# vseib/point-cloud-donkey

Hardware: AMD Instinct MI355X
Metric: objects/sec classified (ModelNet10-like, SHOT-352) (higher is better)
Workload: dtype f32; 1 GPU; configs[1]: ModelNet10-like test split, 16384 pts, 1024 uniform keypoints/object, SHOT-352 (Radius 0.4, LRF 0.3), exact kNN K=1 squared-L2, mean-shift bandwidth 0.6; points_per_object=16384, keypoints_per_object=1024, classes=10, codebook_words=102400, descriptor_dim=352, collective_world_size=1

## Files before the change

### point-cloud-donkey_amd/csrc/codebook.hip

```cpp
#include "common.h"
#include <cstring>
#include <cmath>
#include <limits>

int ism_codebook_split_bf16(ismhip_ctx* ctx, ismhip_codebook* cb, uint32_t absmax_bits);
int ism_codebook_build_pca(ismhip_ctx* ctx, ismhip_codebook* cb);
void ism_codebook_free_pca(ismhip_codebook* cb);

namespace {

__global__ void k_word_norms(const float* __restrict__ words, int n_words, int n_words_pad, int dim_pad, float* __restrict__ norm) {
    const int row = blockIdx.x * 4 + (threadIdx.x >> 6);
    if (row >= n_words_pad) return;
    const int lane = lane_id();
    float s = 0.f;
    for (int c = lane; c < dim_pad; c += 64) { const float v = words[(size_t)row * dim_pad + c]; s += v * v; }
    s = wave_sum_f(s);
    if (lane == 0) norm[row] = row < n_words ? s : __builtin_inff();
}

__global__ void k_sqrt_permuted(const float* __restrict__ src, const uint32_t* __restrict__ perm, int n_words, int dim_pad, float* __restrict__ dst, size_t n) {
    const size_t i = (size_t)blockIdx.x * blockDim.x + threadIdx.x;
    if (i >= n) return;
    const size_t row = i / dim_pad; const int col = (int)(i % dim_pad);
// ... 140 lines not shown
            uint32_t b; memcpy(&b, &words_h[i], 4);
            if (!(words_h[i] >= 0.f)) nonneg = false;
            b &= 0x7fffffffu; amax = b > amax ? b : amax;
        }
        cb->words_nonneg = nonneg;
        int rc = ism_codebook_split_bf16(ctx, cb, amax);
        if (rc != ISMHIP_OK || hipStreamSynchronize(ctx->stream) != hipSuccess) return fail(rc != ISMHIP_OK ? rc : ISMHIP_ERR_HIP, "codebook_create: bf16 split");
        if (!ctx->codebook_light) rc = ism_codebook_build_pca(ctx, cb);
        if (rc != ISMHIP_OK || hipStreamSynchronize(ctx->stream) != hipSuccess) return fail(rc != ISMHIP_OK ? rc : ISMHIP_ERR_HIP, "codebook_create: rotated image");
        if (nonneg && dim > 64 && ctx->knn_hellinger && n_words >= 1024 && !ctx->codebook_light) {
            ismhip_codebook* sh = new ismhip_codebook();
            cb->chi_shadow = sh;
            sh->n_words = n_words; sh->dim = dim; sh->dim_pad = cb->dim_pad; sh->n_words_pad = cb->n_words_pad; sh->n_classes = n_classes;
            if (hipMalloc((void**)&sh->words, wbytes) != hipSuccess || hipMalloc((void**)&sh->word_norm, (size_t)cb->n_words_pad * 4) != hipSuccess)
                return fail(ISMHIP_ERR_NOMEM, "codebook_create: sqrt image");
            std::vector<uint32_t> perm(n_words);
            for (int i = 0; i < n_words; ++i) perm[i] = (uint32_t)i;
            uint64_t st = 0x9E3779B97F4A7C15ull ^ (uint64_t)n_words;
            for (int i = n_words - 1; i > 0; --i) {
                st += 0x9E3779B97F4A7C15ull; uint64_t z = st; z = (z ^ (z >> 30)) * 0xBF58476D1CE4E5B9ull; z = (z ^ (z >> 27)) * 0x94D049BB133111EBull; z ^= z >> 31;
                std::swap(perm[i], perm[(size_t)(z % (uint64_t)(i + 1))]);
            }
            if (!upload(&sh->shadow_perm, perm.data(), (size_t)n_words)) return fail(ISMHIP_ERR_NOMEM, "codebook_create: sqrt image permutation");
            const size_t tot = (size_t)cb->n_words_pad * cb->dim_pad;
            hipLaunchKernelGGL(k_sqrt_permuted, dim3((unsigned)((tot + 255) / 256)), dim3(256), 0, ctx->stream, cb->words, sh->shadow_perm, n_words, cb->dim_pad, sh->words, tot);
            hipLaunchKernelGGL(k_word_norms, dim3((cb->n_words_pad + 3) / 4), dim3(256), 0, ctx->stream, sh->words, n_words, cb->n_words_pad, cb->dim_pad, sh->word_norm);
            if (hipGetLastError() != hipSuccess || hipStreamSynchronize(ctx->stream) != hipSuccess) return fail(ISMHIP_ERR_HIP, "codebook_create: sqrt image kernels");
            std::vector<float> nh(n_words);
            if (hipMemcpy(nh.data(), sh->word_norm, (size_t)n_words * 4, hipMemcpyDeviceToHost) != hipSuccess) return fail(ISMHIP_ERR_HIP, "codebook_create: sqrt norms copy");
            float mx = 0.f;
            for (float v : nh) if (v > mx || v != v) mx = v;
            sh->max_norm2 = mx;
            float amaxf; memcpy(&amaxf, &amax, 4);
            const float samax = sqrtf(amaxf);
            uint32_t samax_bits; memcpy(&samax_bits, &samax, 4);
            rc = ism_codebook_split_bf16(ctx, sh, samax_bits);
            if (rc != ISMHIP_OK || hipStreamSynchronize(ctx->stream) != hipSuccess) return fail(rc != ISMHIP_OK ? rc : ISMHIP_ERR_HIP, "codebook_create: sqrt 16-bit images");
// ... 95 lines not shown
```

### point-cloud-donkey_amd/csrc/common.h

```cpp
#pragma once
#include <hip/hip_runtime.h>
#include <stdint.h>
#include <map>
#include <set>
#include <string>
#include <vector>
#include "../../include/ismhip.h"

#define ISM_WAVE 64

#define ISM_GRID_MAXDIM 32
#define ISM_GRID_MAXCELLS (ISM_GRID_MAXDIM * ISM_GRID_MAXDIM * ISM_GRID_MAXDIM)
#define ISM_GRID_STRIDE (ISM_GRID_MAXCELLS + 1)

#define ISM_GRID_XFRAC 3
struct GridMeta {
    float minv[3];
    float cell[3];
    float inv_cell[3];
    int   dim[3];
    float centroid[3];
    uint32_t n_finite;
};

// ... 47 lines not shown
    float max_norm2 = 0.f;
    float* word_weight = nullptr;
    uint32_t* vote_off = nullptr;
    float* vote_xyz = nullptr;
    float* vote_weight = nullptr;
    float* vote_class_weight = nullptr;
    uint32_t* vote_class = nullptr;
    uint32_t* vote_instance = nullptr;
    float* vote_bbox_quat = nullptr;
    float* vote_bbox_size = nullptr;
    float* class_sigma = nullptr;
    uint32_t* word_class = nullptr;
    ismhip_codebook* chi_shadow = nullptr;
    uint32_t* shadow_perm = nullptr;
    PcaImage pca, pca2;
};

struct TimerAcc {
    std::vector<std::pair<hipEvent_t, hipEvent_t>> pending;
    double ms = 0.0;
    int64_t launches = 0;
};

struct ismhip_ctx {
    int device = 0;
    hipStream_t stream = nullptr;
    bool own_stream = false;
    std::string err;
    bool timers_on = false;
    std::map<std::string, TimerAcc> timers;
    std::vector<hipEvent_t> event_pool;
    struct Slot { void* p = nullptr; size_t bytes = 0; };
    std::map<int, Slot> scratch;
    float* lut_srgb = nullptr;
    float* lut_sxyz = nullptr;
    std::vector<ismhip_cloud*> cloud_pool;
    uint32_t* truncated_d = nullptr;
    uint32_t knn_stats[2] = {0, 0};
    std::set<const void*> attr_done;
    uint32_t knn_stage2_queries = 0;
    bool knn_two_stage = true;
    bool knn_small_tile = false;
    bool knn_join = true;
    bool knn_qpanel2 = true;
    bool knn_qpanel = false;
    bool knn_half = false;
    bool knn_ring32 = false;
    int knn_splits = 0;
    int knn_t = 0;
    int knn_dbg = 0;
    bool knn_no_ring = false;
    bool knn_kb32 = false;
    bool xcd_map = true;
    float grid_xfrac = 0.f;
    int shot_var = 0;
    bool knn_hell_emit = true;
    bool knn_hellinger = true;
    int knn_t1 = 2;
    int knn_pre_step = 32;
    float knn_pre_gamma = 1.0f;
    bool knn_prepass = true;
    int knn_pca_m = -1;
    bool knn_stage2_t4 = false;
    bool codebook_light = false;
    int knn_pca_m2 = -1;
    uint32_t knn_pca_launches = 0;
    uint32_t knn_thr_overflow = 0;
    uint32_t knn_thr_mfma_launches = 0;
    int knn_mode = 0;
};

enum ScratchSlot {
    SCR_KP_OFF = 1, SCR_TIE_LIST, SCR_TIE_REC, SCR_TIE_KEYS, SCR_COUNTERS, SCR_KNN_CAND_IDX, SCR_KNN_CAND_VAL,
    SCR_QNORM, SCR_FPFH_FLAG, SCR_FPFH_LIST, SCR_FPFH_SPFH, SCR_FPFH_LOOKUP, SCR_SLOT_OFF, SCR_CLASS_BW,
    SCR_COMPACT_KEEP, SCR_COMPACT_POS, SCR_OBJ_COUNT, SCR_QPAD, SCR_LRF_COV, SCR_KNN_FLAGS, SCR_KNN_QSPLIT, SCR_MAX_REC, SCR_QNORM2, SCR_KNN_Q2, SCR_KNN_LIST2, SCR_TRAIN, SCR_TRAIN2, SCR_MAX_WORK, SCR_KMEANS, SCR_KNN_CLOCK, SCR_PCA, SCR_KNN_THR0, SCR_KNN_QSQRT, SCR_KNN_HELL_EMIT, SCR_KNN_THR, SCR_KNN_THR2, SCR_TRAIN_ACT
};
// ... 245 lines not shown
```

### point-cloud-donkey_amd/csrc/ctx.hip

```cpp
#include "common.h"
#include <cmath>
#include <cstring>
#include <cstdlib>

extern "C" void ism_cloud_pool_release(ismhip_ctx* ctx);

int ism_set_err(ismhip_ctx* ctx, int code, const std::string& msg) {
    if (ctx) ctx->err = msg;
    return code;
}

void* ism_scratch(ismhip_ctx* ctx, int slot, size_t bytes) {
    if (bytes == 0) bytes = 16;
    auto& s = ctx->scratch[slot];
    if (s.bytes >= bytes) return s.p;
    if (s.p) { (void)hipStreamSynchronize(ctx->stream); (void)hipFree(s.p); s.p = nullptr; s.bytes = 0; }
    size_t want = bytes + bytes / 4;
    void* p = nullptr;
    if (hipMalloc(&p, want) != hipSuccess) { ism_set_err(ctx, ISMHIP_ERR_NOMEM, "scratch hipMalloc failed"); return nullptr; }
    s.p = p; s.bytes = want;
    return p;
}

TimerScope::TimerScope(ismhip_ctx* c, const char* n) : ctx(c), name(n) {
// ... 45 lines not shown
    { const char* e = getenv("ISMHIP_KNN_HALF"); ctx->knn_half = e && e[0] == '1'; }
    { const char* e = getenv("ISMHIP_KNN_RING32"); ctx->knn_ring32 = e && e[0] == '1'; }
    { const char* e = getenv("ISMHIP_KNN_SPLITS"); ctx->knn_splits = e ? atoi(e) : 0; }
    { const char* e = getenv("ISMHIP_KNN_T"); ctx->knn_t = e ? atoi(e) : 0; }
    { const char* e = getenv("ISMHIP_KNN_DBG"); ctx->knn_dbg = e ? atoi(e) : 0; }
    { const char* e = getenv("ISMHIP_KNN_NORING"); ctx->knn_no_ring = e && e[0] == '1'; }
    { const char* e = getenv("ISMHIP_KNN_KB32"); ctx->knn_kb32 = e && e[0] == '1'; }
    { const char* e = getenv("ISMHIP_KNN_HELL_EMIT"); ctx->knn_hell_emit = !(e && e[0] == '0'); }
    { const char* e = getenv("ISMHIP_KNN_HELLINGER"); ctx->knn_hellinger = !(e && e[0] == '0'); }
    { const char* e = getenv("ISMHIP_KNN_T1"); if (e) ctx->knn_t1 = atoi(e); }
    { const char* e = getenv("ISMHIP_KNN_STAGE2_T4"); if (e) ctx->knn_stage2_t4 = atoi(e) != 0; }
    { const char* e = getenv("ISMHIP_KNN_PRE_STEP"); if (e && atoi(e) > 0) ctx->knn_pre_step = atoi(e); }
    { const char* e = getenv("ISMHIP_KNN_PRE_GAMMA"); if (e) ctx->knn_pre_gamma = (float)atof(e); }
    { const char* e = getenv("ISMHIP_KNN_PREPASS"); ctx->knn_prepass = !(e && e[0] == '0'); }
    { const char* e = getenv("ISMHIP_KNN_PCA_M"); ctx->knn_pca_m = e ? atoi(e) : -1; }
    { const char* e = getenv("ISMHIP_KNN_PCA_M2"); ctx->knn_pca_m2 = e ? atoi(e) : -1; }
    { const char* e = getenv("ISMHIP_KNN_TILE128"); ctx->knn_small_tile = e && e[0] == '1'; }
    if (!own) { ctx->stream = (hipStream_t)stream; ctx->own_stream = false; }
    else {
        if (hipStreamCreateWithFlags(&ctx->stream, hipStreamNonBlocking) != hipSuccess) { delete ctx; return ISMHIP_ERR_HIP; }
        ctx->own_stream = true;
    }
    std::vector<float> srgb(256), sxyz(4000);
    for (int i = 0; i < 256; i++) {
        float f = static_cast<float>(i) / 255.0f;
        srgb[i] = (f > 0.04045) ? powf((f + 0.055f) / 1.055f, 2.4f) : f / 12.92f;
    }
    for (int i = 0; i < 4000; i++) {
        float f = static_cast<float>(i) / 4000.0f;
        sxyz[i] = (f > 0.008856) ? static_cast<float>(powf(f, 0.3333f)) : static_cast<float>((7.787 * f) + (16.0 / 116.0));
// ... 94 lines not shown
```

### point-cloud-donkey_amd/csrc/knn.hip

```cpp
#include "common.h"

int ism_pca_rotate_queries(ismhip_ctx* ctx, const ismhip_codebook* cb, const PcaImage* P, const float* q, int nq, int ldq, unsigned short* dst);

namespace {

typedef float f32x16 __attribute__((ext_vector_type(16)));
typedef float f32x4 __attribute__((ext_vector_type(4)));

#define KNN_BM 128
#define KNN_BN 128
#define KNN_BK 32
#define KNN_LDK 36

template <int T>
struct TopT {
    float v[T]; int i[T];
    __device__ __forceinline__ void init() {
#pragma unroll
        for (int t = 0; t < T; ++t) { v[t] = __builtin_inff(); i[t] = -1; }
    }
    __device__ __forceinline__ void push_flat(float x, int idx) {
        bool c[T];
#pragma unroll
        for (int t = 0; t < T; ++t) c[t] = x < v[t];
// ... 1202 lines not shown
        uint32_t ibase = 0;
        if (lane == 0) {
            const uint32_t qs = atomicAdd(&flag_count[0], 1u);
            ibase = atomicAdd(&flag_count[1], (uint32_t)nv);
            qrec[3 * (size_t)qs] = (uint32_t)qi; qrec[3 * (size_t)qs + 1] = ibase; qrec[3 * (size_t)qs + 2] = (uint32_t)nv;
        }
        ibase = __shfl(ibase, 0, 64);
        if (viol) {
            const uint32_t it = ibase + __popcll(vmask & ((1ull << lane) - 1ull));
            items[2 * (size_t)it] = (uint32_t)qi; items[2 * (size_t)it + 1] = (uint32_t)lane;
        }
    }
}
__global__ __launch_bounds__(256) void k_knn_rerank_pca(const float* __restrict__ words, int dim, int dim_pad, int n_words,
                                                        const float* __restrict__ q, int nq, int ldq,
                                                        const int* __restrict__ cand_idx, const float* __restrict__ cand_val, int cand_stride, int n_cand,
                                                        const float* __restrict__ cand_bound, int n_bound, PcaVerify pv,
                                                        int k, int32_t* __restrict__ idx_out, float* __restrict__ dist_out,
                                                        uint32_t* __restrict__ flag_count, uint32_t* __restrict__ qrec, uint32_t* __restrict__ items) {
    const int qi = blockIdx.x * 4 + (threadIdx.x >> 6);
    if (qi >= nq) return;
    const int lane = lane_id();
    const float* qp = q + (size_t)qi * ldq;
    float qn2 = 0.f;
    for (int i = lane; i < dim; i += 64) { const float v = qp[i]; qn2 += v * v; }
    qn2 = wave_sum_f(qn2);
    float qn2h = 0.f;
    {
        const size_t tile = (size_t)(qi >> 8); const int r = qi & 255;
        for (int i = lane; i < pv.nk * 32; i += 64) {
// ... 3 lines not shown
        qn2h = wave_sum_f(qn2h) * pv.inv_sq2;
    }
    const float dlt = pv.d_rel * (sqrtf(qn2) * 1.00001f) + pv.dq_abs + pv.dc;
    const float eps_s = (pv.eps_c2 + pv.dot2 * sqrtf(qn2h * pv.cmax2)) * 1.00001f;
    auto lb_of = [&](float s) -> float {
        float L = qn2h * (1.f - 16.f * KNN_U) + s - eps_s;
        L -= 4.f * KNN_U * (qn2h + fabsf(s));
        if (!(L > 0.f)) return 0.f;
        const float t = sqrtf(L) * (1.f - 4.f * KNN_U) - dlt;
        if (!(t > 0.f)) return 0.f;
        return t * t * pv.inv_sig2 * (1.f - 8.f * KNN_U);
    };
    int id = -1; float av = __builtin_inff();
    if (lane < n_cand) { id = cand_idx[(size_t)qi * cand_stride + lane]; av = cand_val[(size_t)qi * cand_stride + lane]; }
    if (!(id >= 0 && id < n_words)) { id = -1; av = __builtin_inff(); }
    const float lb = id >= 0 ? lb_of(av) : __builtin_inff();
    bool done = id < 0;
    unsigned long long key = ~0ull;
    {
        __shared__ __attribute__((aligned(16))) float s_terms[4][1344];
        float* sT = s_terms[threadIdx.x >> 6];
        float kth = __builtin_inff(); int n_eval = 0;
        for (;;) {
            const float cur = done ? __builtin_inff() : lb;
            const float mn = wave_min_f(cur);
            if (!(mn < __builtin_inff())) break;
            if (n_eval >= k && mn * (1.f - pv.ku) > kth) break;
            const unsigned long long eq = __ballot(!done && cur == mn);
            const int src = __ffsll((long long)eq) - 1;
            const int cid = __shfl(id, src, 64);
// ... 164 lines not shown

#define KNN_FB_UNITS 8192u
__host__ __device__ inline uint32_t knn_fb_parts(uint32_t n_items) {
    if (n_items == 0 || n_items > KNN_FB_UNITS / 2) return 1u;
    const uint32_t p = KNN_FB_UNITS / n_items;
    return p > 256u ? 256u : p;
}
#define KNN_MAX_K 16
#define KNN_FB_MAXJ 84
template <int KM>
__global__ __launch_bounds__(256) void k_knn_fallback(const float* __restrict__ words, int dim, int dim_pad, int n_words,
                                                      const float* __restrict__ q, int ldq, int metric, int k, int tiles_per_split, int n_tiles,
                                                      int tile_rows, int wr_rows ,
                                                      const uint32_t* __restrict__ flag_count, const uint32_t* __restrict__ items,
                                                      const int32_t* __restrict__ idx_in, const float* __restrict__ dist_in,
                                                      unsigned long long* __restrict__ item_out, size_t part_base) {
    __shared__ __attribute__((aligned(16))) float s_terms[4][1344];
    const int lane = threadIdx.x & 63;
    const int g = lane >> 4, l16 = lane & 15;
    const uint32_t n_items = flag_count[1];
    const bool l2 = metric != ISMHIP_METRIC_CHI2;
    const bool lay_all = l2 && wr_rows == -2;
    const bool lay16 = l2 && wr_rows == -1;
    const bool lay16h = l2 && wr_rows == -3;
    const int rows_per_tile = lay_all ? tile_rows : ((lay16 || lay16h) ? 32 : (l2 ? wr_rows / 2 : tile_rows));
    const int nj = dim_pad / 16;
    const uint32_t gw = blockIdx.x * 4 + (threadIdx.x >> 6), nw = gridDim.x * 4;
    const uint32_t P = knn_fb_parts(n_items);
    unsigned long long* outp = P > 1 ? item_out + KM * part_base : item_out;
    for (uint32_t u = gw; u < n_items * P; u += nw) {
        const uint32_t it = u / P, part_i = u % P;
// ... 8 lines not shown
        for (int j = 0; j < KM; ++j) best[j] = ~0ull;
        float thr = __builtin_inff();
        {
            const int id = idx_in[(size_t)qi * k + (k - 1)];
            if (id >= 0) thr = dist_in[(size_t)qi * k + (k - 1)];
        }
        const int steps = (total + 3) / 4;
        const int e_beg = 4 * (int)((long long)steps * part_i / P), e_end = min(total, 4 * (int)((long long)steps * (part_i + 1) / P));
        for (int e0 = e_beg; e0 < e_end; e0 += 4) {
            const int e = e0 + g;
            int r = n_words;
            if (e < e_end) {
                const int tile = mt0 + e / rows_per_tile, y = e % rows_per_tile;
                const int x = lay_all ? y : ((lay16 || lay16h) ? (wr * 128 + ((y >> 2) << 4) + (fq << 2) + (y & 3)) : (l2 ? (wr * wr_rows + (((y >> 2) << 3) | (h << 2) | (y & 3))) : y));
                r = tile * tile_rows + x;
            }
            float part = 0.f;
            if (r < n_words) {
                const float* wp = words + (size_t)r * dim_pad;
                if (!l2) { for (int j = 0; j < nj; ++j) { const int i = l16 + 16 * j; const float a = i < dim ? qp[i] : 0.f, c = wp[i], sm = a + c, df = a - c; part += sm > 0.f ? df * df / sm : 0.f; } }
                else { for (int j = 0; j < nj; ++j) { const int i = l16 + 16 * j; const float df = (i < dim ? qp[i] : 0.f) - wp[i]; part += df * df; } }
            }
#pragma unroll
            for (int o = 8; o > 0; o >>= 1) part += __shfl_xor(part, o, 64);
            const bool hit = r < n_words && !(part > thr * 1.0001f + 1e-30f);
            unsigned long long hm = __ballot(hit && l16 == 0);
            while (hm) {
                const int src = __ffsll((long long)hm) - 1; hm &= hm - 1;
                const int rr = __shfl(r, src, 64);
                const float d = wave_functor(metric, qp, words + (size_t)rr * dim_pad, dim, lane, s_terms[threadIdx.x >> 6]);
// ... 79 lines not shown
    const float a = d3[i * 3], b = d3[i * 3 + 1], c = d3[i * 3 + 2];
    int id = -1; float dd = __builtin_nanf("");
    if (i2 < 0) {
        if (i0 >= 0) { id = i0; dd = a; }
    } else {
        const uint32_t c0 = word_class[i0], c1 = word_class[i1], c2 = word_class[i2];
        if (c0 == c1 && c0 == c2) { id = i0; dd = a; }
        else if (c0 == c1 && c0 != c2) { if (a / c < thr) { id = i0; dd = a; } }
        else if (c0 != c1 && c1 == c2) { if (a / b >= thr) { id = i1; dd = b; } }
        else if (c0 != c1 && c1 != c2) { if (a / b < thr) { id = i0; dd = a; } }
    }
    idx_out[i] = id; dist_out[i] = dd;
}

struct KnnStage1 { uint32_t* flag_count; uint32_t* qrec; };
template <int T>
int run_knn(ismhip_ctx* ctx, const ismhip_codebook* cb, int metric, int nq, const float* q, int k,
            int32_t* idx_out, float* dist_out, KnnStage1* stage1 = nullptr, const char* tname = nullptr, bool many_splits = false, int use_pca = 0 , const float* hell_q = nullptr) {
    const bool hell = hell_q != nullptr && metric == ISMHIP_METRIC_CHI2 && cb->chi_shadow;
    const ismhip_codebook* xb = hell ? cb->chi_shadow : cb;
    const int cmetric = hell ? ISMHIP_METRIC_L2SQ : metric;
    if (cb->dim_pad / 16 > KNN_FB_MAXJ) return ism_set_err(ctx, ISMHIP_ERR_UNSUPPORTED, "knn: descriptor longer than 1344 not built");
    const float* qq = q; int ldq = cb->dim;
    if (cb->dim_pad != cb->dim) {
        float* qpad = (float*)ism_scratch(ctx, SCR_QPAD, (size_t)nq * cb->dim_pad * sizeof(float));
        if (!qpad) return ISMHIP_ERR_NOMEM;
        const size_t tot = (size_t)nq * cb->dim_pad;
        hipLaunchKernelGGL(k_pad_rows, dim3((unsigned)((tot + 255) / 256)), dim3(256), 0, ctx->stream, q, nq, cb->dim, qpad, cb->dim_pad);
        ISM_CHECK_LAUNCH(ctx, "k_pad_rows");
        qq = qpad; ldq = cb->dim_pad;
// ... 109 lines not shown
                    default: break;
                } else
                switch (ctx->knn_dbg) {
                    case 1: rk = (const void*)k_knn_l2_ring<T, 1>; break;  case 3: rk = (const void*)k_knn_l2_ring<T, 3>; break;
                    case 5: rk = (const void*)k_knn_l2_ring<T, 5>; break;  case 7: rk = (const void*)k_knn_l2_ring<T, 7>; break;
                    case 9: rk = (const void*)k_knn_l2_ring<T, 9>; break;  case 13: rk = (const void*)k_knn_l2_ring<T, 13>; break;
                    case 15: rk = (const void*)k_knn_l2_ring<T, 15>; break; case 11: rk = (const void*)k_knn_l2_ring<T, 11>; break;
                    case 21: rk = (const void*)k_knn_l2_ring<T, 21>; break; case 513: rk = (const void*)k_knn_l2_ring<T, 513>; break; case 256: rk = (const void*)k_knn_l2_ring<T, 256>; break; case 64: rk = (const void*)k_knn_l2_ring<T, 64>; break; case 128: rk = (const void*)k_knn_l2_ring<T, 128>; break; case 192: rk = (const void*)k_knn_l2_ring<T, 192>; break; case 53: rk = (const void*)k_knn_l2_ring<T, 53>; break; case 37: rk = (const void*)k_knn_l2_ring<T, 37>; break;
                    default: break;
                }
#endif
                const size_t rlds = qpanel2 ? (size_t)4 * 256 * RG_KB * sizeof(u16) + 4 * 256 * sizeof(float) + 8 * 4 * 64 * sizeof(float) + (size_t)ring_nk * 256 * RG_KB * sizeof(u16)
                                  : qpanel ? (size_t)4 * 256 * RG_KB * sizeof(u16) + 4 * 256 * sizeof(float) + 8 * 2 * 64 * sizeof(float) + (size_t)ring_nk * 128 * RG_KB * sizeof(u16)
                                  : half ? (size_t)3 * (128 + 256) * RG_KB * sizeof(u16) + 4 * 256 * sizeof(float)
                                         : (size_t)RG_STAGES * RG_STAGE_HALVES * sizeof(u16) + 4 * RG_BM * sizeof(float) + 8 * 4 * 64 * sizeof(float);
                if (ctx->knn_dbg || !ctx->attr_done.count(rk)) {
                    ISM_HIP(ctx, hipFuncSetAttribute(rk, hipFuncAttributeMaxDynamicSharedMemorySize, (int)rlds));
                    ctx->attr_done.insert(rk);
                }
                const float* osc = (const float*)(qsc + 1);
                const float* word_norm;
                if (pca) { wh = PI.f16t; osc = PI.osc; word_norm = PI.cn_scaled; }
                else {
                    float* cn_scaled = (float*)ism_scratch(ctx, SCR_QNORM2, ((size_t)cb->n_words_pad + 256) * sizeof(float));
                    if (!cn_scaled) return ISMHIP_ERR_NOMEM;
                    hipLaunchKernelGGL(k_scale_norms, dim3((cb->n_words_pad + 255) / 256), dim3(256), 0, ctx->stream, xb->word_norm, cb->n_words_pad, osc, cn_scaled);
                    ISM_CHECK_LAUNCH(ctx, "k_scale_norms");
                    word_norm = cn_scaled;
                }
                int n_tiles_m = cb->n_words_pad / BM, ld16 = cb->ld16, k_steps = pca ? PI.m / 16 : (cb->dim + 15) / 16, nq_ = nq, tps = tiles_per_split, nsp = n_splits, ncand = n_cand, nb = n_bound;
                const u16* qh_ = q_hi;
                unsigned int* clock = nullptr;
                if (ring16 && ctx->knn_join) {
                    clock = (unsigned int*)ism_scratch(ctx, SCR_KNN_CLOCK, 8 * 64 * sizeof(unsigned int));
                    if (!clock) return ISMHIP_ERR_NOMEM;
                    ISM_HIP(ctx, hipMemsetAsync(clock, 0, 8 * 64 * sizeof(unsigned int), ctx->stream));
                }
                const float* thr_init = nullptr; float* thr_out = nullptr; int tile_step = 1;
                if (stage1 && ring16 && !half && !qpanel && ctx->knn_prepass && n_tiles_m >= 128 && ctx->knn_dbg == 0 && !(pca && PI.resid2 <= 0.f)) {
                    float* thr0 = (float*)ism_scratch(ctx, SCR_KNN_THR0, (size_t)((nq + 255) / 256 * 256) * sizeof(float));
                    if (!thr0) return ISMHIP_ERR_NOMEM;
                    const void* pk = (const void*)k_knn_l2_ring16<T, 2, 0, 0, 1>;
                    if (!ctx->attr_done.count(pk)) { ISM_HIP(ctx, hipFuncSetAttribute(pk, hipFuncAttributeMaxDynamicSharedMemorySize, (int)rlds)); ctx->attr_done.insert(pk); }
                    int one = 1, all = n_tiles_m, step = ctx->knn_pre_step; unsigned int* noclk = nullptr; const float* noinit = nullptr;
                    float relax = 0.f;
                    if (pca) relax = -ctx->knn_pre_gamma * 2.0f * PI.resid2 * (PI.sq * PI.sc * 0.5f);
                    void* pargs[] = {&wh, &word_norm, &n_tiles_m, &ld16, &k_steps, &qh_, &nq_, &osc, &all, &one, &cand_val, &cand_idx, &ncand, &cand_bound, &nb, &noclk, &noinit, &thr0, &step, &relax};
                    ISM_HIP(ctx, hipLaunchKernel(pk, dim3(8 * ((n_qt + 7) / 8)), dim3(512), pargs, rlds, ctx->stream));
                    ISM_CHECK_LAUNCH(ctx, "k_knn_l2_ring16<pre>");
                    thr_init = thr0;
                }
                float no_relax = 0.f;
                void* rargs[] = {&wh, &word_norm, &n_tiles_m, &ld16, &k_steps, &qh_, &nq_, &osc, &tps, &nsp, &cand_val, &cand_idx, &ncand, &cand_bound, &nb, &clock, &thr_init, &thr_out, &tile_step, &no_relax};
                ISM_HIP(ctx, hipLaunchKernel(rk, grid, dim3(half ? 256 : 512), rargs, rlds, ctx->stream));
                ISM_CHECK_LAUNCH(ctx, "k_knn_l2_ring");
            } else {
            (void)ai;
            if (!ctx->attr_done.count(kern)) { ISM_HIP(ctx, hipFuncSetAttribute(kern, hipFuncAttributeMaxDynamicSharedMemorySize, (int)lds)); ctx->attr_done.insert(kern); }
            const float* word_norm = xb->word_norm; const float* osc = (const float*)(qsc + 1);
            int n_tiles_m = cb->n_words_pad / BM, ld16 = cb->ld16, k_steps = (cb->dim + 15) / 16, nq_ = nq, tps = tiles_per_split, nsp = n_splits, ncand = n_cand, nb = n_bound;
            const u16* qh_ = q_hi; const u16* ql_ = q_lo;
            const float* no_tau = nullptr; uint32_t* no_u = nullptr; int no_cap = 0;
            void* args[] = {&wh, &wl, &word_norm, &n_tiles_m, &ld16, &k_steps, &qh_, &ql_, &nq_, &osc, &tps, &nsp, &cand_val, &cand_idx, &ncand, &cand_bound, &nb, &no_tau, &no_u, &no_u, &no_cap};
            ISM_HIP(ctx, hipLaunchKernel(kern, grid, dim3(big_tile ? 512 : 256), args, lds, ctx->stream));
            ISM_CHECK_LAUNCH(ctx, "k_knn_l2_mfma16");
            }
        } else if (cmetric == ISMHIP_METRIC_L2SQ) {
            const int n_qt = (nq + KNN_BN - 1) / KNN_BN;
            hipLaunchKernelGGL(k_knn_l2_mfma<T>, dim3(8 * ((n_qt + 7) / 8) * n_splits), dim3(256), 0, ctx->stream, cb->words, cb->word_norm,
                               cb->n_words_pad / KNN_BM, cb->dim_pad, qq, nq, ldq, tiles_per_split, n_splits, cand_val, cand_idx, n_cand,
                               cand_bound, n_bound, std::min(16, cb->dim - (cb->dim_pad / KNN_BK - 1) * KNN_BK));
            ISM_CHECK_LAUNCH(ctx, "k_knn_l2_mfma");
        } else {
// ... 26 lines not shown
    vp.cn_acc = mode == 0 ? 1.01f * (float)(cb->dim_pad + 1) * 1.1920929e-07f : 0.f;
    {
    TimerScope trr(ctx, "knn_rerank");
    if (pca) {
        PcaVerify pv;
        const float acc_rel = 1.01f * (float)PI.m * 1.1920929e-07f;
        pv.qimg = q_hi; pv.nk = ring_nk; pv.inv_sq2 = 1.0f / (PI.sq * PI.sq);
        pv.inv_sig2 = PI.inv_sig2; pv.d_rel = PI.d_rel; pv.dq_abs = PI.dq_abs;
        pv.dc = (PI.d_rel * sqrtf(cb->max_norm2) + PI.dc_abs) * 1.00001f;
        pv.cmax2 = PI.cmax2;
        const float fq = 6.103515625e-05f / PI.sq, fc = 6.103515625e-05f / PI.sc, sm = sqrtf((float)PI.m);
        pv.eps_c2 = (17.f * KNN_U + 1.01f * (float)(PI.m + 1) * 1.1920929e-07f) * PI.cmax2 + 2.02f * (sm * fq * sqrtf(PI.cmax2) + sm * sm * fq * fc);
        pv.dot2 = 2.f * acc_rel + 2.f * KNN_U + 2.02f * sm * fc / sqrtf(PI.cmax2);
        pv.ku = vp.ku;
        hipLaunchKernelGGL(k_knn_rerank_pca, dim3((nq + 3) / 4), dim3(256), 0, ctx->stream, cb->words, cb->dim, cb->dim_pad, cb->n_words,
                           qq, nq, ldq, cand_idx, cand_val, n_cand, n_cand, cand_bound, n_bound, pv, k, idx_out, dist_out, flag_count, qrec, items);
    } else if (hell) {
        hipLaunchKernelGGL(k_knn_rerank_hell, dim3((nq + 3) / 4), dim3(256), 0, ctx->stream, cb->words, cb->dim, cb->dim_pad, cb->n_words,
                           qq, nq, ldq, hell_q, xb->shadow_perm, cand_idx, cand_val, n_cand, n_cand, cand_bound, n_bound, vp, k, idx_out, dist_out, flag_count, qrec, items);
    } else
    hipLaunchKernelGGL(k_knn_rerank, dim3((nq + 3) / 4), dim3(256), 0, ctx->stream, cb->words, cb->dim, cb->dim_pad, cb->n_words,
                       qq, nq, ldq, metric, cand_idx, cand_val, n_cand, n_cand, cand_bound, n_bound, vp, k, idx_out, dist_out, flag_count, qrec, items);
    ISM_CHECK_LAUNCH(ctx, "k_knn_rerank");
    }
    if (stage1) { stage1->flag_count = flag_count; stage1->qrec = qrec; return ISMHIP_OK; }
    {
        TimerScope ts(ctx, "knn_fallback");
        const int fb_tps = merged ? cb->n_words_pad / BM : tiles_per_split, fb_lay = merged ? -2 : (half ? -3 : (ring16 ? -1 : wr_rows));
        if (k <= 4) hipLaunchKernelGGL(k_knn_fallback<4>, dim3(1024), dim3(256), 0, ctx->stream, cb->words, cb->dim, cb->dim_pad, cb->n_words, qq, ldq, metric, k,
                                       fb_tps, cb->n_words_pad / BM, BM, fb_lay, flag_count, items, idx_out, dist_out, item_out, q_items);
        else hipLaunchKernelGGL(k_knn_fallback<KNN_MAX_K>, dim3(1024), dim3(256), 0, ctx->stream, cb->words, cb->dim, cb->dim_pad, cb->n_words, qq, ldq, metric, k,
                                fb_tps, cb->n_words_pad / BM, BM, fb_lay, flag_count, items, idx_out, dist_out, item_out, q_items);
        ISM_CHECK_LAUNCH(ctx, "k_knn_fallback");
        if (k <= 4) hipLaunchKernelGGL(k_knn_fallback_merge<4>, dim3(256), dim3(256), 0, ctx->stream, k, flag_count, qrec, item_out, q_items, idx_out, dist_out);
        else hipLaunchKernelGGL(k_knn_fallback_merge<KNN_MAX_K>, dim3(256), dim3(256), 0, ctx->stream, k, flag_count, qrec, item_out, q_items, idx_out, dist_out);
        ISM_CHECK_LAUNCH(ctx, "k_knn_fallback_merge");
    }
    if (ctx->timers_on) ISM_HIP(ctx, hipMemcpyAsync(ctx->knn_stats, flag_count, 8, hipMemcpyDeviceToHost, ctx->stream));
    return ISMHIP_OK;
}

__global__ __launch_bounds__(256) void k_knn_gather_flagged(const uint32_t* __restrict__ qrec, int n2, const float* __restrict__ q, int dim,
                                                            float* __restrict__ q2, uint32_t* __restrict__ list2) {
    const int i = blockIdx.x;
    if (i >= n2) return;
    const uint32_t qi = qrec[3 * (size_t)i];
    if (threadIdx.x == 0) list2[i] = qi;
// ... 573 lines not shown
```

### point-cloud-donkey_amd/csrc/pca.hip

```cpp
#include "common.h"
#include <cmath>
#include <cstring>
#include <algorithm>
#include <numeric>

namespace {

typedef float f32x16 __attribute__((ext_vector_type(16)));
typedef float f32x4 __attribute__((ext_vector_type(4)));
typedef unsigned short u16;

#define SM_ROWS 64
__global__ __launch_bounds__(256) void k_second_moment(const float* __restrict__ w, int n_rows, int ld, int rows_per_chunk, int nb, float* __restrict__ part) {
    __shared__ float sA[SM_ROWS][33], sB[SM_ROWS][33];
    int bi = 0, rem = blockIdx.x;
    while (rem >= nb - bi) { rem -= nb - bi; ++bi; }
    const int bj = bi + rem;
    const int tx = threadIdx.x & 15, ty = threadIdx.x >> 4;
    const int r_beg = blockIdx.y * rows_per_chunk, r_end = min(n_rows, r_beg + rows_per_chunk);
    float a00 = 0.f, a01 = 0.f, a10 = 0.f, a11 = 0.f;
    for (int r0 = r_beg; r0 < r_end; r0 += SM_ROWS) {
        __syncthreads();
        for (int e = threadIdx.x; e < SM_ROWS * 32; e += 256) {
            const int rr = e >> 5, c = e & 31, r = r0 + rr;
// ... 4 lines not shown
#pragma unroll 8
        for (int rr = 0; rr < SM_ROWS; ++rr) {
            const float x0 = sA[rr][2 * ty], x1 = sA[rr][2 * ty + 1], y0 = sB[rr][2 * tx], y1 = sB[rr][2 * tx + 1];
            a00 = fmaf(x0, y0, a00); a01 = fmaf(x0, y1, a01); a10 = fmaf(x1, y0, a10); a11 = fmaf(x1, y1, a11);
        }
    }
    const int dimp = nb * 32;
    float* o = part + (size_t)blockIdx.y * dimp * dimp;
    o[(size_t)(bi * 32 + 2 * ty) * dimp + bj * 32 + 2 * tx] = a00;     o[(size_t)(bi * 32 + 2 * ty) * dimp + bj * 32 + 2 * tx + 1] = a01;
    o[(size_t)(bi * 32 + 2 * ty + 1) * dimp + bj * 32 + 2 * tx] = a10; o[(size_t)(bi * 32 + 2 * ty + 1) * dimp + bj * 32 + 2 * tx + 1] = a11;
}

#define ROT_LD 36
template <int NT>
__global__ __launch_bounds__(256, 2) void k_rotate_f16t(const float* __restrict__ x, int n, int ldx, int kdim,
                                                         const float* __restrict__ rmat, int m, float scale, u16* __restrict__ dst) {
    extern __shared__ __attribute__((aligned(16))) float rot_smem[];
    float* sX = rot_smem;
    float* sR = rot_smem + 128 * ROT_LD;
    const int tid = threadIdx.x, lane = tid & 63, wv = tid >> 6;
    const int r32 = lane & 31, h = lane >> 5;
    const int nct = m >> 5;
    const size_t row0 = (size_t)blockIdx.x * 128;
    f32x16 acc[NT];
#pragma unroll
    for (int t = 0; t < NT; ++t)
#pragma unroll
        for (int e = 0; e < 16; ++e) acc[t][e] = 0.f;
    const int srow = tid >> 3, scol = (tid & 7) * 4;
    for (int k0 = 0; k0 < kdim; k0 += 32) {
        __syncthreads();
#pragma unroll
        for (int i = 0; i < 4; ++i) {
            size_t r = row0 + srow + 32 * i; r = r < (size_t)n ? r : (size_t)n - 1;
            *(f32x4*)(sX + (srow + 32 * i) * ROT_LD + scol) = *(const f32x4*)(x + r * ldx + k0 + scol);
        }
#pragma unroll
        for (int i = 0; i < NT; ++i)
            if (i < nct) *(f32x4*)(sR + (srow + 32 * i) * ROT_LD + scol) = *(const f32x4*)(rmat + (size_t)(srow + 32 * i) * kdim + k0 + scol);
        __syncthreads();
        f32x4 fb[4];
        const float* pb = sX + (wv * 32 + r32) * ROT_LD + h * 16;
#pragma unroll
        for (int v = 0; v < 4; ++v) fb[v] = *(const f32x4*)(pb + 4 * v);
#pragma unroll
        for (int t = 0; t < NT; ++t) {
            if (t >= nct) continue;
            f32x4 fa[4];
            const float* pa = sR + (t * 32 + r32) * ROT_LD + h * 16;
// ... 67 lines not shown
    w.resize(n);
    for (int i = 0; i < n; ++i) w[i] = A[(size_t)i * n + i];
}

float f16_scale_of_bound(float bound) {
    uint32_t b; memcpy(&b, &bound, 4);
    const int e = (int)((b >> 23) & 255u);
    if (e == 0 || e == 255) return 1.0f;
    int k = 13 - (e - 127);
    k = k > 40 ? 40 : (k < -40 ? -40 : k);
    const uint32_t u = (uint32_t)(127 + k) << 23;
    float f; memcpy(&f, &u, 4);
    return f;
}

int launch_rotate(ismhip_ctx* ctx, const float* x, int n, int ldx, int kdim, const float* rmat, int m, float scale, u16* dst) {
    const int nct = m / 32;
    const void* kern = nct <= 4 ? (const void*)k_rotate_f16t<4> : nct <= 6 ? (const void*)k_rotate_f16t<6> : (const void*)k_rotate_f16t<8>;
    const int nt = nct <= 4 ? 4 : nct <= 6 ? 6 : 8;
    const size_t lds = (size_t)(128 + nt * 32) * ROT_LD * sizeof(float);
    if (!ctx->attr_done.count(kern)) { ISM_HIP(ctx, hipFuncSetAttribute(kern, hipFuncAttributeMaxDynamicSharedMemorySize, (int)lds)); ctx->attr_done.insert(kern); }
    const unsigned blocks = (unsigned)((((size_t)n + 255) / 256 * 256) / 128);
    void* args[] = {&x, &n, &ldx, &kdim, &rmat, &m, &scale, &dst};
    ISM_HIP(ctx, hipLaunchKernel(kern, dim3(blocks), dim3(256), args, lds, ctx->stream));
    ISM_CHECK_LAUNCH(ctx, "k_rotate_f16t");
    return ISMHIP_OK;
}

}

int ism_pca_rotate_queries(ismhip_ctx* ctx, const ismhip_codebook* cb, const PcaImage* P, const float* q, int nq, int ldq, unsigned short* dst) {
    return launch_rotate(ctx, q, nq, ldq, cb->dim_pad, P->R, P->m, P->sq, dst);
}

static int build_image(ismhip_ctx* ctx, ismhip_codebook* cb, PcaImage& P, const std::vector<float>& R, int m, double energy, double trace) {
    const int dp = cb->dim_pad;
    P.m = 0;
    double e2 = 0, fro2 = 0;
// ... 8 lines not shown
    P.sq = f16_scale_of_bound((float)(2.002 * sig * cmax));
    const double gamma = 1.01 * dp * 1.1920929e-07;
    P.d_rel = (float)(1.001 * (gamma * fro + 4.8828125e-04 * (sig + gamma * fro)));
    P.dq_abs = (float)(1.001 * std::sqrt((double)m) * 6.103515625e-05 / P.sq);
    P.dc_abs = (float)(1.001 * std::sqrt((double)m) * 6.103515625e-05 / P.sc);
    P.inv_sig2 = (float)((1.0 / sig2) * (1.0 - 1e-6));
    P.energy = (float)energy;
    P.resid2 = (float)((1.0 - energy) * trace / (double)cb->n_words);
    const int nk = m / 32, n_tiles = cb->n_words_pad / 256;
    if (hipMalloc((void**)&P.R, R.size() * sizeof(float)) != hipSuccess) return ism_set_err(ctx, ISMHIP_ERR_NOMEM, "codebook rotation matrix");
    ISM_HIP(ctx, hipMemcpy(P.R, R.data(), R.size() * sizeof(float), hipMemcpyHostToDevice));
    if (hipMalloc((void**)&P.f16t, (size_t)n_tiles * nk * 8192 * sizeof(u16)) != hipSuccess) return ism_set_err(ctx, ISMHIP_ERR_NOMEM, "codebook rotated f16 image");
    if (hipMalloc((void**)&P.cn_scaled, ((size_t)cb->n_words_pad + 256) * sizeof(float) + 16) != hipSuccess) return ism_set_err(ctx, ISMHIP_ERR_NOMEM, "codebook rotated norms");
    P.osc = P.cn_scaled + cb->n_words_pad + 256;
    P.m = m;
    int rc = launch_rotate(ctx, cb->words, cb->n_words_pad, dp, dp, P.R, m, P.sc, P.f16t);
    if (rc != ISMHIP_OK) { P.m = 0; return rc; }
    float* sumsq_d = (float*)ism_scratch(ctx, SCR_PCA, (size_t)cb->n_words_pad * sizeof(float));
    if (!sumsq_d) { P.m = 0; return ISMHIP_ERR_NOMEM; }
    ISM_HIP(ctx, hipMemsetAsync(P.cn_scaled, 0, ((size_t)cb->n_words_pad + 256) * sizeof(float), ctx->stream));
    const float cn_factor = P.sq / (2.0f * P.sc);
    hipLaunchKernelGGL(k_f16t_norms, dim3((cb->n_words_pad + 3) / 4), dim3(256), 0, ctx->stream, P.f16t, cb->n_words_pad, cb->n_words, nk, cn_factor, sumsq_d, P.cn_scaled);
    ISM_CHECK_LAUNCH(ctx, "k_f16t_norms");
    std::vector<float> ss(cb->n_words);
    ISM_HIP(ctx, hipMemcpyAsync(ss.data(), sumsq_d, (size_t)cb->n_words * sizeof(float), hipMemcpyDeviceToHost, ctx->stream));
    const float osc = -2.0f / (P.sq * P.sc);
    ISM_HIP(ctx, hipMemcpyAsync(P.osc, &osc, sizeof(float), hipMemcpyHostToDevice, ctx->stream));
    ISM_HIP(ctx, hipStreamSynchronize(ctx->stream));
    float mx = 0.f;
    for (float v : ss) mx = v > mx || v != v ? v : mx;
    P.cmax2 = mx / (P.sc * P.sc) * 1.00001f;
// ... 37 lines not shown
    for (int i = 0; i < dp; ++i) for (int j = i + 1; j < dp; ++j) { const double v = i / 32 == j / 32 ? 0.5 * (S[(size_t)i * dp + j] + S[(size_t)j * dp + i]) : S[(size_t)i * dp + j]; S[(size_t)i * dp + j] = v; S[(size_t)j * dp + i] = v; }
    for (int i = 0; i < dp; ++i) trace += S[(size_t)i * dp + i];
    if (!(trace > 0) || !std::isfinite(trace)) return ISMHIP_OK;
    jacobi_eig(dp, S, V, w);
    std::vector<int> order(dp); std::iota(order.begin(), order.end(), 0);
    std::stable_sort(order.begin(), order.end(), [&](int a, int b) { return w[a] > w[b]; });
    w_sorted.resize(dp); V_sorted.resize((size_t)dp * dp);
    for (int j = 0; j < dp; ++j) { w_sorted[j] = w[order[j]]; std::copy(V.begin() + (size_t)order[j] * dp, V.begin() + (size_t)(order[j] + 1) * dp, V_sorted.begin() + (size_t)j * dp); }
    const int m_cap = std::min(256, dp);
    double cum = 0; energy = 0;
    if (ctx->knn_pca_m > 0) {
        m = std::max(64, std::min(m_cap, (ctx->knn_pca_m + 31) / 32 * 32));
        for (int i = 0; i < m; ++i) energy += w[order[i]];
        energy /= trace;
    } else {
        for (int i = 0; i < dp && !m; ++i) { cum += w[order[i]]; if ((i + 1) % 32 == 0 && i + 1 >= 64 && cum >= 0.97 * trace) { m = i + 1; energy = cum / trace; } }
        if (m == 0 || m > m_cap || m + 64 > dp) return ISMHIP_OK;
    }
    R.assign((size_t)m * dp, 0.f);
    for (int j = 0; j < m; ++j) for (int c = 0; c < dp; ++c) R[(size_t)j * dp + c] = c < cb->dim ? (float)V[(size_t)order[j] * dp + c] : 0.f;
    }
    int rc = build_image(ctx, cb, cb->pca, R, m, energy, trace);
    if (rc != ISMHIP_OK || cb->pca.m == 0 || identity || ctx->knn_pca_m2 == 0) return rc;
    int m2 = 0; double cum2 = 0, energy2 = 0;
    if (ctx->knn_pca_m2 > 0) m2 = std::max(m + 32, std::min(std::min(256, dp), (ctx->knn_pca_m2 + 31) / 32 * 32));
    for (int i = 0; i < dp; ++i) {
        cum2 += w_sorted[i];
        if (m2 == 0 && (i + 1) % 32 == 0 && i + 1 >= m + 64 && cum2 >= 0.997 * trace) m2 = i + 1;
        if (m2 && i + 1 == m2) energy2 = cum2 / trace;
    }
    if (m2 == 0 || m2 > std::min(256, dp) || (m2 + 64 > dp && ctx->knn_pca_m2 < 0)) return ISMHIP_OK;
    std::vector<float> R2((size_t)m2 * dp, 0.f);
    for (int j = 0; j < m2; ++j) for (int c2 = 0; c2 < dp; ++c2) R2[(size_t)j * dp + c2] = c2 < cb->dim ? (float)V_sorted[(size_t)j * dp + c2] : 0.f;
    return build_image(ctx, cb, cb->pca2, R2, m2, energy2, trace);
}

void ism_codebook_free_pca(ismhip_codebook* cb) {
    for (PcaImage* P : {&cb->pca, &cb->pca2}) {
        if (P->R) (void)hipFree(P->R);
        if (P->f16t) (void)hipFree(P->f16t);
        if (P->cn_scaled) (void)hipFree(P->cn_scaled);
        *P = PcaImage();
    }
}
```

Baseline: 18320 objects/s.

## Randomly permute PCA-rotated codebook rows and relax PCA energy and prepass gamma

Builds the PCA-rotated 16-bit codebook image with a pseudo-random row permutation, the same way the sqrt shadow image is already built. The rerank and fallback kernels map candidate indices back through the permutation. Spreading similar words across tiles is meant to tighten per-tile bounds and cut stage-2 work. It also lowers the PCA energy threshold (fewer rotated dims), halves the prepass relaxation gamma, and tracks the dynamic LDS attribute per kernel by size. The permuted rows add a gather load and make the screen looser, which may send more queries to verification or fallback.

```diff
diff --git a/point-cloud-donkey_amd/csrc/codebook.hip b/point-cloud-donkey_amd/csrc/codebook.hip
--- a/point-cloud-donkey_amd/csrc/codebook.hip
+++ b/point-cloud-donkey_amd/csrc/codebook.hip
@@ -178,13 +178,7 @@
             sh->n_words = n_words; sh->dim = dim; sh->dim_pad = cb->dim_pad; sh->n_words_pad = cb->n_words_pad; sh->n_classes = n_classes;
             if (hipMalloc((void**)&sh->words, wbytes) != hipSuccess || hipMalloc((void**)&sh->word_norm, (size_t)cb->n_words_pad * 4) != hipSuccess)
                 return fail(ISMHIP_ERR_NOMEM, "codebook_create: sqrt image");
-            std::vector<uint32_t> perm(n_words);
-            for (int i = 0; i < n_words; ++i) perm[i] = (uint32_t)i;
-            uint64_t st = 0x9E3779B97F4A7C15ull ^ (uint64_t)n_words;
-            for (int i = n_words - 1; i > 0; --i) {
-                st += 0x9E3779B97F4A7C15ull; uint64_t z = st; z = (z ^ (z >> 30)) * 0xBF58476D1CE4E5B9ull; z = (z ^ (z >> 27)) * 0x94D049BB133111EBull; z ^= z >> 31;
-                std::swap(perm[i], perm[(size_t)(z % (uint64_t)(i + 1))]);
-            }
+            const std::vector<uint32_t> perm = ism_row_permutation(n_words);
             if (!upload(&sh->shadow_perm, perm.data(), (size_t)n_words)) return fail(ISMHIP_ERR_NOMEM, "codebook_create: sqrt image permutation");
             const size_t tot = (size_t)cb->n_words_pad * cb->dim_pad;
             hipLaunchKernelGGL(k_sqrt_permuted, dim3((unsigned)((tot + 255) / 256)), dim3(256), 0, ctx->stream, cb->words, sh->shadow_perm, n_words, cb->dim_pad, sh->words, tot);
diff --git a/point-cloud-donkey_amd/csrc/common.h b/point-cloud-donkey_amd/csrc/common.h
--- a/point-cloud-donkey_amd/csrc/common.h
+++ b/point-cloud-donkey_amd/csrc/common.h
@@ -85,7 +85,20 @@
     ismhip_codebook* chi_shadow = nullptr;
     uint32_t* shadow_perm = nullptr;
     PcaImage pca, pca2;
-};
+    uint32_t* pca_perm = nullptr;
+};
+
+static inline std::vector<uint32_t> ism_row_permutation(int n) {
+    std::vector<uint32_t> perm(n);
+    for (int i = 0; i < n; ++i) perm[i] = (uint32_t)i;
+    uint64_t st = 0x9E3779B97F4A7C15ull ^ (uint64_t)n;
+    for (int i = n - 1; i > 0; --i) {
+        st += 0x9E3779B97F4A7C15ull; uint64_t z = st; z = (z ^ (z >> 30)) * 0xBF58476D1CE4E5B9ull; z = (z ^ (z >> 27)) * 0x94D049BB133111EBull; z ^= z >> 31;
+        const size_t j = (size_t)(z % (uint64_t)(i + 1));
+        const uint32_t t = perm[i]; perm[i] = perm[j]; perm[j] = t;
+    }
+    return perm;
+}
 
 struct TimerAcc {
     std::vector<std::pair<hipEvent_t, hipEvent_t>> pending;
@@ -109,6 +122,7 @@
     uint32_t* truncated_d = nullptr;
     uint32_t knn_stats[2] = {0, 0};
     std::set<const void*> attr_done;
+    std::map<const void*, int> attr_lds;
     uint32_t knn_stage2_queries = 0;
     bool knn_two_stage = true;
     bool knn_small_tile = false;
@@ -129,8 +143,9 @@
     bool knn_hellinger = true;
     int knn_t1 = 2;
     int knn_pre_step = 32;
-    float knn_pre_gamma = 1.0f;
+    float knn_pre_gamma = 0.5f;
     bool knn_prepass = true;
+    bool knn_pca_permute = true;
     int knn_pca_m = -1;
     bool knn_stage2_t4 = false;
     bool codebook_light = false;
diff --git a/point-cloud-donkey_amd/csrc/ctx.hip b/point-cloud-donkey_amd/csrc/ctx.hip
--- a/point-cloud-donkey_amd/csrc/ctx.hip
+++ b/point-cloud-donkey_amd/csrc/ctx.hip
@@ -83,6 +83,7 @@
     { const char* e = getenv("ISMHIP_KNN_PRE_GAMMA"); if (e) ctx->knn_pre_gamma = (float)atof(e); }
     { const char* e = getenv("ISMHIP_KNN_PREPASS"); ctx->knn_prepass = !(e && e[0] == '0'); }
     { const char* e = getenv("ISMHIP_KNN_PCA_M"); ctx->knn_pca_m = e ? atoi(e) : -1; }
+    { const char* e = getenv("ISMHIP_KNN_PCA_PERMUTE"); ctx->knn_pca_permute = !(e && e[0] == '0'); }
     { const char* e = getenv("ISMHIP_KNN_PCA_M2"); ctx->knn_pca_m2 = e ? atoi(e) : -1; }
     { const char* e = getenv("ISMHIP_KNN_TILE128"); ctx->knn_small_tile = e && e[0] == '1'; }
     if (!own) { ctx->stream = (hipStream_t)stream; ctx->own_stream = false; }
diff --git a/point-cloud-donkey_amd/csrc/knn.hip b/point-cloud-donkey_amd/csrc/knn.hip
--- a/point-cloud-donkey_amd/csrc/knn.hip
+++ b/point-cloud-donkey_amd/csrc/knn.hip
@@ -1240,6 +1240,7 @@
 }
 __global__ __launch_bounds__(256) void k_knn_rerank_pca(const float* __restrict__ words, int dim, int dim_pad, int n_words,
                                                         const float* __restrict__ q, int nq, int ldq,
+                                                        const uint32_t* __restrict__ perm ,
                                                         const int* __restrict__ cand_idx, const float* __restrict__ cand_val, int cand_stride, int n_cand,
                                                         const float* __restrict__ cand_bound, int n_bound, PcaVerify pv,
                                                         int k, int32_t* __restrict__ idx_out, float* __restrict__ dist_out,
@@ -1273,6 +1274,7 @@
     int id = -1; float av = __builtin_inff();
     if (lane < n_cand) { id = cand_idx[(size_t)qi * cand_stride + lane]; av = cand_val[(size_t)qi * cand_stride + lane]; }
     if (!(id >= 0 && id < n_words)) { id = -1; av = __builtin_inff(); }
+    else if (perm) id = (int)perm[id];
     const float lb = id >= 0 ? lb_of(av) : __builtin_inff();
     bool done = id < 0;
     unsigned long long key = ~0ull;
@@ -1467,7 +1469,7 @@
                                                       int tile_rows, int wr_rows ,
                                                       const uint32_t* __restrict__ flag_count, const uint32_t* __restrict__ items,
                                                       const int32_t* __restrict__ idx_in, const float* __restrict__ dist_in,
-                                                      unsigned long long* __restrict__ item_out, size_t part_base) {
+                                                      unsigned long long* __restrict__ item_out, size_t part_base, const uint32_t* __restrict__ perm) {
     __shared__ __attribute__((aligned(16))) float s_terms[4][1344];
     const int lane = threadIdx.x & 63;
     const int g = lane >> 4, l16 = lane & 15;
@@ -1506,6 +1508,7 @@
                 const int tile = mt0 + e / rows_per_tile, y = e % rows_per_tile;
                 const int x = lay_all ? y : ((lay16 || lay16h) ? (wr * 128 + ((y >> 2) << 4) + (fq << 2) + (y & 3)) : (l2 ? (wr * wr_rows + (((y >> 2) << 3) | (h << 2) | (y & 3))) : y));
                 r = tile * tile_rows + x;
+                if (perm && r < n_words) r = (int)perm[r];
             }
             float part = 0.f;
             if (r < n_words) {
@@ -1615,6 +1618,12 @@
 }
 
 struct KnnStage1 { uint32_t* flag_count; uint32_t* qrec; };
+static int knn_raise_lds(ismhip_ctx* ctx, const void* kern, size_t bytes) {
+    int& have = ctx->attr_lds[kern];
+    if ((int)bytes > have) { ISM_HIP(ctx, hipFuncSetAttribute(kern, hipFuncAttributeMaxDynamicSharedMemorySize, (int)bytes)); have = (int)bytes; }
+    return ISMHIP_OK;
+}
+
 template <int T>
 int run_knn(ismhip_ctx* ctx, const ismhip_codebook* cb, int metric, int nq, const float* q, int k,
             int32_t* idx_out, float* dist_out, KnnStage1* stage1 = nullptr, const char* tname = nullptr, bool many_splits = false, int use_pca = 0 , const float* hell_q = nullptr) {
@@ -1754,10 +1763,7 @@
                                   : qpanel ? (size_t)4 * 256 * RG_KB * sizeof(u16) + 4 * 256 * sizeof(float) + 8 * 2 * 64 * sizeof(float) + (size_t)ring_nk * 128 * RG_KB * sizeof(u16)
                                   : half ? (size_t)3 * (128 + 256) * RG_KB * sizeof(u16) + 4 * 256 * sizeof(float)
                                          : (size_t)RG_STAGES * RG_STAGE_HALVES * sizeof(u16) + 4 * RG_BM * sizeof(float) + 8 * 4 * 64 * sizeof(float);
-                if (ctx->knn_dbg || !ctx->attr_done.count(rk)) {
-                    ISM_HIP(ctx, hipFuncSetAttribute(rk, hipFuncAttributeMaxDynamicSharedMemorySize, (int)rlds));
-                    ctx->attr_done.insert(rk);
-                }
+                if (const int rc = knn_raise_lds(ctx, rk, rlds)) return rc;
                 const float* osc = (const float*)(qsc + 1);
                 const float* word_norm;
                 if (pca) { wh = PI.f16t; osc = PI.osc; word_norm = PI.cn_scaled; }
@@ -1781,12 +1787,13 @@
                     float* thr0 = (float*)ism_scratch(ctx, SCR_KNN_THR0, (size_t)((nq + 255) / 256 * 256) * sizeof(float));
                     if (!thr0) return ISMHIP_ERR_NOMEM;
                     const void* pk = (const void*)k_knn_l2_ring16<T, 2, 0, 0, 1>;
-                    if (!ctx->attr_done.count(pk)) { ISM_HIP(ctx, hipFuncSetAttribute(pk, hipFuncAttributeMaxDynamicSharedMemorySize, (int)rlds)); ctx->attr_done.insert(pk); }
+                    const size_t plds = (size_t)RG_STAGES * RG_STAGE_HALVES * sizeof(u16) + 4 * RG_BM * sizeof(float) + 8 * 4 * 64 * sizeof(float);
+                    if (const int rc = knn_raise_lds(ctx, pk, plds)) return rc;
                     int one = 1, all = n_tiles_m, step = ctx->knn_pre_step; unsigned int* noclk = nullptr; const float* noinit = nullptr;
                     float relax = 0.f;
                     if (pca) relax = -ctx->knn_pre_gamma * 2.0f * PI.resid2 * (PI.sq * PI.sc * 0.5f);
                     void* pargs[] = {&wh, &word_norm, &n_tiles_m, &ld16, &k_steps, &qh_, &nq_, &osc, &all, &one, &cand_val, &cand_idx, &ncand, &cand_bound, &nb, &noclk, &noinit, &thr0, &step, &relax};
-                    ISM_HIP(ctx, hipLaunchKernel(pk, dim3(8 * ((n_qt + 7) / 8)), dim3(512), pargs, rlds, ctx->stream));
+                    ISM_HIP(ctx, hipLaunchKernel(pk, dim3(8 * ((n_qt + 7) / 8)), dim3(512), pargs, plds, ctx->stream));
                     ISM_CHECK_LAUNCH(ctx, "k_knn_l2_ring16<pre>");
                     thr_init = thr0;
                 }
@@ -1796,7 +1803,7 @@
                 ISM_CHECK_LAUNCH(ctx, "k_knn_l2_ring");
             } else {
             (void)ai;
-            if (!ctx->attr_done.count(kern)) { ISM_HIP(ctx, hipFuncSetAttribute(kern, hipFuncAttributeMaxDynamicSharedMemorySize, (int)lds)); ctx->attr_done.insert(kern); }
+            if (const int rc = knn_raise_lds(ctx, kern, lds)) return rc;
             const float* word_norm = xb->word_norm; const float* osc = (const float*)(qsc + 1);
             int n_tiles_m = cb->n_words_pad / BM, ld16 = cb->ld16, k_steps = (cb->dim + 15) / 16, nq_ = nq, tps = tiles_per_split, nsp = n_splits, ncand = n_cand, nb = n_bound;
             const u16* qh_ = q_hi; const u16* ql_ = q_lo;
@@ -1853,7 +1860,7 @@
         pv.dot2 = 2.f * acc_rel + 2.f * KNN_U + 2.02f * sm * fc / sqrtf(PI.cmax2);
         pv.ku = vp.ku;
         hipLaunchKernelGGL(k_knn_rerank_pca, dim3((nq + 3) / 4), dim3(256), 0, ctx->stream, cb->words, cb->dim, cb->dim_pad, cb->n_words,
-                           qq, nq, ldq, cand_idx, cand_val, n_cand, n_cand, cand_bound, n_bound, pv, k, idx_out, dist_out, flag_count, qrec, items);
+                           qq, nq, ldq, cb->pca_perm, cand_idx, cand_val, n_cand, n_cand, cand_bound, n_bound, pv, k, idx_out, dist_out, flag_count, qrec, items);
     } else if (hell) {
         hipLaunchKernelGGL(k_knn_rerank_hell, dim3((nq + 3) / 4), dim3(256), 0, ctx->stream, cb->words, cb->dim, cb->dim_pad, cb->n_words,
                            qq, nq, ldq, hell_q, xb->shadow_perm, cand_idx, cand_val, n_cand, n_cand, cand_bound, n_bound, vp, k, idx_out, dist_out, flag_count, qrec, items);
@@ -1866,10 +1873,11 @@
     {
         TimerScope ts(ctx, "knn_fallback");
         const int fb_tps = merged ? cb->n_words_pad / BM : tiles_per_split, fb_lay = merged ? -2 : (half ? -3 : (ring16 ? -1 : wr_rows));
+        const uint32_t* fb_perm = pca ? cb->pca_perm : nullptr;
         if (k <= 4) hipLaunchKernelGGL(k_knn_fallback<4>, dim3(1024), dim3(256), 0, ctx->stream, cb->words, cb->dim, cb->dim_pad, cb->n_words, qq, ldq, metric, k,
-                                       fb_tps, cb->n_words_pad / BM, BM, fb_lay, flag_count, items, idx_out, dist_out, item_out, q_items);
+                                       fb_tps, cb->n_words_pad / BM, BM, fb_lay, flag_count, items, idx_out, dist_out, item_out, q_items, fb_perm);
         else hipLaunchKernelGGL(k_knn_fallback<KNN_MAX_K>, dim3(1024), dim3(256), 0, ctx->stream, cb->words, cb->dim, cb->dim_pad, cb->n_words, qq, ldq, metric, k,
-                                fb_tps, cb->n_words_pad / BM, BM, fb_lay, flag_count, items, idx_out, dist_out, item_out, q_items);
+                                fb_tps, cb->n_words_pad / BM, BM, fb_lay, flag_count, items, idx_out, dist_out, item_out, q_items, fb_perm);
         ISM_CHECK_LAUNCH(ctx, "k_knn_fallback");
         if (k <= 4) hipLaunchKernelGGL(k_knn_fallback_merge<4>, dim3(256), dim3(256), 0, ctx->stream, k, flag_count, qrec, item_out, q_items, idx_out, dist_out);
         else hipLaunchKernelGGL(k_knn_fallback_merge<KNN_MAX_K>, dim3(256), dim3(256), 0, ctx->stream, k, flag_count, qrec, item_out, q_items, idx_out, dist_out);
diff --git a/point-cloud-donkey_amd/csrc/pca.hip b/point-cloud-donkey_amd/csrc/pca.hip
--- a/point-cloud-donkey_amd/csrc/pca.hip
+++ b/point-cloud-donkey_amd/csrc/pca.hip
@@ -42,7 +42,8 @@
 #define ROT_LD 36
 template <int NT>
 __global__ __launch_bounds__(256, 2) void k_rotate_f16t(const float* __restrict__ x, int n, int ldx, int kdim,
-                                                         const float* __restrict__ rmat, int m, float scale, u16* __restrict__ dst) {
+                                                         const float* __restrict__ rmat, int m, float scale, u16* __restrict__ dst,
+                                                         const uint32_t* __restrict__ perm, int n_perm) {
     extern __shared__ __attribute__((aligned(16))) float rot_smem[];
     float* sX = rot_smem;
     float* sR = rot_smem + 128 * ROT_LD;
@@ -61,6 +62,7 @@
 #pragma unroll
         for (int i = 0; i < 4; ++i) {
             size_t r = row0 + srow + 32 * i; r = r < (size_t)n ? r : (size_t)n - 1;
+            if (perm && r < (size_t)n_perm) r = perm[r];
             *(f32x4*)(sX + (srow + 32 * i) * ROT_LD + scol) = *(const f32x4*)(x + r * ldx + k0 + scol);
         }
 #pragma unroll
@@ -158,14 +160,15 @@
     return f;
 }
 
-int launch_rotate(ismhip_ctx* ctx, const float* x, int n, int ldx, int kdim, const float* rmat, int m, float scale, u16* dst) {
+int launch_rotate(ismhip_ctx* ctx, const float* x, int n, int ldx, int kdim, const float* rmat, int m, float scale, u16* dst,
+                  const uint32_t* perm = nullptr, int n_perm = 0) {
     const int nct = m / 32;
     const void* kern = nct <= 4 ? (const void*)k_rotate_f16t<4> : nct <= 6 ? (const void*)k_rotate_f16t<6> : (const void*)k_rotate_f16t<8>;
     const int nt = nct <= 4 ? 4 : nct <= 6 ? 6 : 8;
     const size_t lds = (size_t)(128 + nt * 32) * ROT_LD * sizeof(float);
     if (!ctx->attr_done.count(kern)) { ISM_HIP(ctx, hipFuncSetAttribute(kern, hipFuncAttributeMaxDynamicSharedMemorySize, (int)lds)); ctx->attr_done.insert(kern); }
     const unsigned blocks = (unsigned)((((size_t)n + 255) / 256 * 256) / 128);
-    void* args[] = {&x, &n, &ldx, &kdim, &rmat, &m, &scale, &dst};
+    void* args[] = {&x, &n, &ldx, &kdim, &rmat, &m, &scale, &dst, &perm, &n_perm};
     ISM_HIP(ctx, hipLaunchKernel(kern, dim3(blocks), dim3(256), args, lds, ctx->stream));
     ISM_CHECK_LAUNCH(ctx, "k_rotate_f16t");
     return ISMHIP_OK;
@@ -204,7 +207,7 @@
     if (hipMalloc((void**)&P.cn_scaled, ((size_t)cb->n_words_pad + 256) * sizeof(float) + 16) != hipSuccess) return ism_set_err(ctx, ISMHIP_ERR_NOMEM, "codebook rotated norms");
     P.osc = P.cn_scaled + cb->n_words_pad + 256;
     P.m = m;
-    int rc = launch_rotate(ctx, cb->words, cb->n_words_pad, dp, dp, P.R, m, P.sc, P.f16t);
+    int rc = launch_rotate(ctx, cb->words, cb->n_words_pad, dp, dp, P.R, m, P.sc, P.f16t, cb->pca_perm, cb->n_words);
     if (rc != ISMHIP_OK) { P.m = 0; return rc; }
     float* sumsq_d = (float*)ism_scratch(ctx, SCR_PCA, (size_t)cb->n_words_pad * sizeof(float));
     if (!sumsq_d) { P.m = 0; return ISMHIP_ERR_NOMEM; }
@@ -272,11 +275,17 @@
         for (int i = 0; i < m; ++i) energy += w[order[i]];
         energy /= trace;
     } else {
-        for (int i = 0; i < dp && !m; ++i) { cum += w[order[i]]; if ((i + 1) % 32 == 0 && i + 1 >= 64 && cum >= 0.97 * trace) { m = i + 1; energy = cum / trace; } }
+        const double share = ctx->knn_pca_permute ? 0.95 : 0.97;
+        for (int i = 0; i < dp && !m; ++i) { cum += w[order[i]]; if ((i + 1) % 32 == 0 && i + 1 >= 64 && cum >= share * trace) { m = i + 1; energy = cum / trace; } }
         if (m == 0 || m > m_cap || m + 64 > dp) return ISMHIP_OK;
     }
     R.assign((size_t)m * dp, 0.f);
     for (int j = 0; j < m; ++j) for (int c = 0; c < dp; ++c) R[(size_t)j * dp + c] = c < cb->dim ? (float)V[(size_t)order[j] * dp + c] : 0.f;
+    }
+    if (!identity && ctx->knn_pca_permute) {
+        const std::vector<uint32_t> perm = ism_row_permutation(cb->n_words);
+        if (hipMalloc((void**)&cb->pca_perm, perm.size() * sizeof(uint32_t)) != hipSuccess) return ism_set_err(ctx, ISMHIP_ERR_NOMEM, "codebook rotated image permutation");
+        ISM_HIP(ctx, hipMemcpy(cb->pca_perm, perm.data(), perm.size() * sizeof(uint32_t), hipMemcpyHostToDevice));
     }
     int rc = build_image(ctx, cb, cb->pca, R, m, energy, trace);
     if (rc != ISMHIP_OK || cb->pca.m == 0 || identity || ctx->knn_pca_m2 == 0) return rc;
@@ -300,4 +309,6 @@
         if (P->cn_scaled) (void)hipFree(P->cn_scaled);
         *P = PcaImage();
     }
-}
+    if (cb->pca_perm) (void)hipFree(cb->pca_perm);
+    cb->pca_perm = nullptr;
+}
```

Result: faster. 18580 objects/s (median of 6 runs) (+1.4%).
